# JoelTankard/web-rwkv-gguf

Measured on AMD Instinct MI355X. Metric: tokens/sec RWKV-7 1.5B Q4_K_M decode @1 GPU; achieved HBM GB/s vs roofline, higher is better.
Workload: dtype f16; 1 GPU; RWKV-7 World 1.5B Q4_K_M (Q4_K matrices, Q6_K head, F16 LoRA) batch=1 greedy decode, fused kernels under hipGraph; decode_engine=on, streams_per_gpu=1, pipelines_per_gpu=1, streams=1, parallelism=single

## Files before the change

### web-rwkv-gguf_amd/csrc/wrk_v7_engine.h

```cpp
#pragma once
#include <stdint.h>

#include "wrk_internal.h"

namespace wrk {

constexpr int ENG_K1_JOBS = 7;
constexpr uint32_t ENG_NO_HEAD = 0xffffffffu;

struct EngJob {
    uint32_t rows, row_bytes, f16;
    uint32_t act, mix;
    uint32_t wg0, nwg, rows_per_wg;
    uint32_t gbase;
    uint32_t headed;
};

struct EngShape {
    uint32_t D, F, H, nwg;
    uint32_t rw, ra, rg, rv;
    uint32_t rb_d, rb_f;
    uint32_t rb_w2, rb_a2, rb_g2, rb_v2;
    EngJob k1[ENG_K1_JOBS];
    uint32_t k3_rpw, k5_rpw, k6_rpw;
    uint32_t lds_slot1, lds_slot5, lds_slot6, lds_slot3, lds_xraw0, lds_xraw1, lds_xs, lds_ln, lds_misc, lds_total;
    uint32_t g_x, g_k1, g_o, g_x1, g_k, g_total, g_aux;
    float ln_eps, gn_eps, l2_eps;
    uint32_t layer_begin, layer_end, rescale;
    uint32_t batch, state_rows;
    uint32_t x_from_granules;
};

struct EngLayer {
    const uint8_t *w_r, *w_k, *w_v, *w1, *a1, *g1, *v1;
    const uint8_t *w2, *a2, *g2, *v2;
    const uint8_t *w_o, *ffn_k, *ffn_v;
};
enum { ENG_V_LN1W, ENG_V_LN1B, ENG_V_LN2W, ENG_V_LN2B, ENG_V_MIX0, ENG_V_W0 = ENG_V_MIX0 + 6, ENG_V_A0, ENG_V_V0, ENG_V_RK, ENG_V_KK, ENG_V_KA,
       ENG_V_GNW, ENG_V_GNB, ENG_V_FFNXK, ENG_NV };
enum { ENG_S_O = ENG_K1_JOBS, ENG_S_FK, ENG_S_FV, ENG_NS = 16 };

struct EngArgs {
    EngShape S;
    const EngLayer* layers;
    const void* vecs;
    const float* scal;
    unsigned long long* gran;
    const void* x_in;
    const uint32_t* x_row;
    void* x_out;
    void* v_first;
    float* state;
    uint32_t num_batch;
    uint32_t* fail;
    unsigned long long* stamps;
    uint32_t stamp_layer;
};
constexpr int ENG_STAMPS = 32;

constexpr __host__ __device__ uint32_t eng_wave_pairs(uint32_t pairs, uint32_t ncw, uint32_t wave) {
    const uint32_t simd_rank = (wave + 4u - (ncw + 2u) % 4u) % 4u;
    return pairs / ncw + ((wave / 4u) * 4u + simd_rank < pairs % ncw ? 1u : 0u);
}
constexpr __host__ __device__ uint32_t eng_wave_first_pair(uint32_t pairs, uint32_t ncw, uint32_t wave) {
    const uint32_t extra = pairs % ncw, g4 = (wave / 4u) * 4u;
    uint32_t first = wave * (pairs / ncw) + (extra < g4 ? extra : g4);
    for (uint32_t w = g4; w < wave; ++w) first += eng_wave_pairs(pairs, ncw, w) - pairs / ncw;
    return first;
}
constexpr __host__ __device__ void eng_wave_rows(uint32_t nrows, uint32_t ncw, uint32_t wave, uint32_t& begin, uint32_t& end) {
    const uint32_t pairs = (nrows + 1u) / 2u;
    const uint32_t first = eng_wave_first_pair(pairs, ncw, wave), last = first + eng_wave_pairs(pairs, ncw, wave);
    begin = 2u * first < nrows ? 2u * first : nrows;
    end = 2u * last < nrows ? 2u * last : nrows;
}
constexpr bool eng_wave_rows_ok(uint32_t ncw) {
    for (uint32_t nrows = 0; nrows <= 128; nrows += 2) {
        const uint32_t pairs = nrows / 2, most = (pairs + ncw - 1) / ncw;
// ... 33 lines not shown
```

### web-rwkv-gguf_amd/csrc/wrk_v7_engine.hip

```cpp
#include "wrk_device.h"
#include "wrk_v7.h"
#include "wrk_dmv_body.h"
#include "wrk_v7_engine.h"
#include "wrk_lora_dev.h"

#include <algorithm>
#include <string>

namespace wrk {

#define ENG_LDS __attribute__((address_space(3)))
typedef ENG_LDS unsigned char lds_u8;

#define ENG_BAR() asm volatile("s_waitcnt lgkmcnt(0)\n\ts_barrier" ::: "memory")

constexpr uint32_t ENG_SPIN_MAX = 1u << 21;

__device__ __forceinline__ uint32_t eng_tag(uint32_t layer, uint32_t stage) { return layer * 8u + stage + 1u; }

__device__ __forceinline__ void eng_store_granule(unsigned long long* g, uint32_t tag, uint32_t payload) {
    __hip_atomic_store(g, ((unsigned long long)tag << 32) | payload, __ATOMIC_RELAXED, __HIP_MEMORY_SCOPE_AGENT);
}
__device__ __forceinline__ uint32_t pack_h2(float a, float b) {
    const f16x2 h = {(f16)a, (f16)b};
// ... 105 lines not shown
    const f16x8 z = {0, 0, 0, 0, 0, 0, 0, 0};
    r.v[0] = r.v[1] = r.v[2] = r.v[3] = z;
    r.s[0] = r.s[1] = 0.0f;
    uint32_t lo, hi;
    chunk_xoff<KIND>(c, lo, hi);
    r.v[0] = *(const ENG_LDS f16x8*)(x + lo);
    if (KIND != WRK_MAT_F16) {
        r.v[1] = *(const ENG_LDS f16x8*)(x + lo + 8);
        r.v[2] = *(const ENG_LDS f16x8*)(x + hi);
        r.v[3] = *(const ENG_LDS f16x8*)(x + hi + 8);
    }
    return r;
}

template <int MAXCH>
__device__ __forceinline__ float eng_lora_dot(const f16x8 (&w)[MAXCH], const ENG_LDS f16* aux, uint32_t rank, uint32_t part) {
    float acc = 0.0f;
#pragma unroll
    for (int n = 0; n < MAXCH; ++n) {
        const uint32_t c = part * 8 + 32 * n;
        if (c < rank) {
            const f16x8 x = *(const ENG_LDS f16x8*)(aux + c);
            acc = __builtin_amdgcn_fdot2(__builtin_shufflevector(w[n], w[n], 0, 1), __builtin_shufflevector(x, x, 0, 1), acc, false);
            acc = __builtin_amdgcn_fdot2(__builtin_shufflevector(w[n], w[n], 2, 3), __builtin_shufflevector(x, x, 2, 3), acc, false);
            acc = __builtin_amdgcn_fdot2(__builtin_shufflevector(w[n], w[n], 4, 5), __builtin_shufflevector(x, x, 4, 5), acc, false);
            acc = __builtin_amdgcn_fdot2(__builtin_shufflevector(w[n], w[n], 6, 7), __builtin_shufflevector(x, x, 6, 7), acc, false);
        }
    }
    acc += dpp_f32<0xB1>(acc);
    acc += dpp_f32<0x4E>(acc);
    return acc;
}

struct EngFin {
    uint32_t act;
    float scale;
    const ENG_LDS f16* res;
    float post;
};
__device__ __forceinline__ float eng_finish(const EngFin& f, uint32_t row, float v) {
    float o = act_apply(f.act, v * f.scale);
    if (f.res) o = r16(o) + (float)f.res[row];
    return o;
}

template <int KIND, bool R16, int XI, int RB, class GIDX>
__device__ __forceinline__ void eng_rows(const lds_u8* slot, uint32_t row_bytes, uint32_t K, const ENG_LDS f16* xs, uint32_t row0, uint32_t r_begin,
                                         uint32_t r_end, const EngFin& fin, ENG_LDS uint32_t* pub, unsigned long long* gran, uint32_t tag, GIDX gidx,
                                         uint32_t lane) {
    if (r_begin >= r_end) return;
    const uint32_t kpad = (K + 15u) & ~15u;
    const uint32_t nch = num_chunks<KIND>(K, kpad);
    XRegs x[1][XI];
#pragma unroll
    for (int ci = 0; ci < XI; ++ci) {
        const uint32_t c = lane + 64u * ci;
        x[0][ci] = lds_x<KIND>(xs, min(c, nch - 1));
        if (c >= nch) {
            const f16x8 z = {0, 0, 0, 0, 0, 0, 0, 0};
            x[0][ci].v[0] = x[0][ci].v[1] = x[0][ci].v[2] = x[0][ci].v[3] = z;
        }
        x_sums<KIND>(x[0][ci]);
    }
    static_assert(RB == 2 || RB == 4, "rows per batch");
    constexpr bool PAD = XI > 1;
    for (uint32_t ri = r_begin; ri < r_end; ri += RB) {
// ... 3 lines not shown
        for (int rb = 0; rb < RB; ++rb) {
            const lds_u8* rowp = slot + (size_t)min(ri + rb, r_end - 1) * row_bytes;
#pragma unroll
            for (int ci = 0; ci < XI; ++ci) raw[rb][ci] = lds_raw<KIND>(rowp, K, min(lane + 64u * ci, nch - 1));
        }
        float v[4] = {0.0f, 0.0f, 0.0f, 0.0f};
#pragma unroll
        for (int rb = 0; rb < RB; ++rb)
            if (rb < 2 || whole) {
                float acc[1] = {0.0f};
#pragma unroll
                for (int ci = 0; ci < XI; ++ci) dot_raw_tokens<KIND, R16, 1, XI>(raw[rb][ci], min(lane + 64u * ci, nch - 1), x, ci, acc);
                v[rb] = wave_sum(acc[0]);
            }
        if (lane < RB / 2) {
            const uint32_t ra = ri + 2 * lane;
            if (ra < r_end) {
                const float o0 = eng_finish(fin, row0 + ra, lane ? v[2] : v[0]) * fin.post;
                const float o1 = eng_finish(fin, row0 + ra + 1, lane ? v[3] : v[1]) * fin.post;
                if (pub) pub[ra >> 1] = pack_h2(o0, o1);
                else eng_store_granule(gran + gidx(row0 + ra), tag, pack_h2(o0, o1));
            }
        }
    }
}

template <class GIDX>
__device__ __forceinline__ void eng_publish(const ENG_LDS uint32_t* pub, uint32_t nrows, uint32_t row0, unsigned long long* gran, uint32_t tag, GIDX gidx,
                                            uint32_t lane) {
    for (uint32_t i = lane; 2 * i < nrows; i += 64) eng_store_granule(gran + gidx(row0 + 2 * i), tag, pub[i]);
}

template <int VPT>
__device__ __forceinline__ void eng_ln_mix(bool active, const ENG_LDS f16* xraw, ENG_LDS f16* xs, ENG_LDS f16* ln_out, ENG_LDS float* red, uint32_t K, float eps,
                                           const f16x8 (&wv)[VPT], const f16x8 (&bv)[VPT], const f16x8 (&mv)[VPT], const f32x4 (&pv)[VPT][2],
                                           uint32_t tid, uint32_t lane, uint32_t wave) {
    const uint32_t nvec = K >> 3;
    f16x8 xv[VPT];
    float c0 = 0.0f;
    if (active) {
#pragma unroll
        for (int v = 0; v < VPT; ++v) xv[v] = *(const ENG_LDS f16x8*)(xraw + min(tid + 256u * v, nvec - 1) * 8);
        c0 = (float)xraw[0];
        float s1 = 0.0f, s2 = 0.0f;
#pragma unroll
        for (int v = 0; v < VPT; ++v)
            if (tid + 256u * v < nvec)
#pragma unroll
                for (int e = 0; e < 8; ++e) { const float dl = (float)xv[v][e] - c0; s1 += dl; s2 = __builtin_fmaf(dl, dl, s2); }
        s1 = wave_sum(s1);
        s2 = wave_sum(s2);
        if (lane == 0) { red[wave] = s1; red[4 + wave] = s2; }
    }
    ENG_BAR();
    if (active) {
        const float a1 = (red[0] + red[1]) + (red[2] + red[3]);
        const float a2 = (red[4] + red[5]) + (red[6] + red[7]);
        const float md = a1 / (float)K;
        const float mean = c0 + md;
        const float dev = 1.0f / sqrtf(fmaxf(a2 / (float)K - md * md, 0.0f) + eps);
#pragma unroll
        for (int v = 0; v < VPT; ++v) {
            const uint32_t i = tid + 256u * v;
            if (i >= nvec) continue;
            f16x8 yv, o;
#pragma unroll
            for (int e = 0; e < 8; ++e) {
                yv[e] = (f16)__builtin_fmaf(((float)xv[v][e] - mean) * dev, (float)wv[v][e], (float)bv[v][e]);
                o[e] = (f16)wgsl_mix((float)yv[e], pv[v][e >> 2][e & 3], (float)mv[v][e]);
            }
            *(ENG_LDS f16x8*)(xs + i * 8) = o;
            *(ENG_LDS f16x8*)(ln_out + i * 8) = yv;
        }
    }
    ENG_BAR();
}

constexpr int ENG_LN_BARRIERS = 2;
constexpr int ENG_K1_BARRIERS = 2 + ENG_LN_BARRIERS;
constexpr int ENG_K2_BARRIERS = 6;
constexpr int ENG_K2_CHECKED = 2;
constexpr int ENG_K3_BARRIERS = 2;
constexpr int ENG_K5_BARRIERS = 3 + ENG_LN_BARRIERS;
constexpr int ENG_K6_BARRIERS = 3;
template <int N>
__device__ __forceinline__ void eng_replay() {
#pragma unroll
    for (int i = 0; i < N; ++i) ENG_BAR();
}
template <int XD, bool R16, int QK, int NCW>
__global__ void __launch_bounds__((NCW + 2) * 64) v7_engine_kernel(const EngArgs A, const uint32_t* __restrict__ wg_head) {
    extern __shared__ __attribute__((aligned(16))) unsigned char eng_smem_generic[];
    lds_u8* smem = (lds_u8*)eng_smem_generic;
// ... 134 lines not shown
            ENG_BAR();
            if (*abort_flag) break;
            eng_replay<ENG_K6_BARRIERS - 1>();
            ENG_FLUSH(l);
        }
        return;
    }

    constexpr int VPT = XD;
    constexpr int S64 = 64;
    constexpr int MAXU = (16 + NCW - 1) / NCW;
    const uint32_t nvec = D >> 3;
    const float eps = S.ln_eps;
    const bool ln_wave = wave < 4;
    const uint32_t c0 = is_head ? head * S64 : 0u;
    float vfirst_keep = 0.0f;
    if (is_head && S.layer_begin > 0 && wave == 0) vfirst_keep = (float)((const f16*)A.v_first)[c0 + (tid_all & 63u)];

    unsigned long long clk0 = 0, rt0 = 0;
    if (A.stamps && wg == 0 && tid_all == 0) { clk0 = __builtin_amdgcn_s_memtime(); rt0 = __builtin_amdgcn_s_memrealtime(); }
    for (uint32_t l = S.layer_begin; l < S.layer_end; ++l) {
        uint32_t tid = tid_all;
        asm volatile("" : "+v"(tid));
        const uint32_t lane = tid & 63u;
        float* lst = layer_state(l);
        const bool layer0 = l == 0;
        const f16* lv_base = (const f16*)A.vecs + (size_t)l * ENG_NV * D;
        auto lvec = [&](uint32_t idx) { return lv_base + (size_t)idx * D; };
        const float* scl = A.scal + (size_t)l * ENG_NS;
        const float sc_k1 = scl[j1 < ENG_K1_JOBS ? j1 : 0u], sc_o = scl[ENG_S_O], sc_fk = scl[ENG_S_FK], sc_fv = scl[ENG_S_FV];

        f16x8 wv[VPT], bv[VPT], mv[VPT];
        f32x4 pv[VPT][2];
        if (ln_wave) {
            const f16* mixp = lvec(ENG_V_MIX0 + (j1 < ENG_K1_JOBS ? S.k1[j1].mix : 0u));
#pragma unroll
            for (int v = 0; v < VPT; ++v) {
                const uint32_t i = min(tid + 256u * v, nvec - 1);
                wv[v] = *(const f16x8*)(lvec(ENG_V_LN1W) + i * 8);
                bv[v] = *(const f16x8*)(lvec(ENG_V_LN1B) + i * 8);
                mv[v] = *(const f16x8*)(mixp + i * 8);
                pv[v][0] = *(const f32x4*)(lst + i * 8);
                pv[v][1] = *(const f32x4*)(lst + i * 8 + 4);
            }
        }

        auto request_k5 = [&]() {
            if (ln_wave) {
                float* rowf = lst + (size_t)(srows - 1) * D;
    #pragma unroll
                for (int v = 0; v < VPT; ++v) {
                    const uint32_t i = min(tid + 256u * v, nvec - 1);
                    wv[v] = *(const f16x8*)(lvec(ENG_V_LN2W) + i * 8);
                    bv[v] = *(const f16x8*)(lvec(ENG_V_LN2B) + i * 8);
                    mv[v] = *(const f16x8*)(lvec(ENG_V_FFNXK) + i * 8);
                    pv[v][0] = *(const f32x4*)(rowf + i * 8);
                    pv[v][1] = *(const f32x4*)(rowf + i * 8 + 4);
                }
            }
        };
        if (!is_head) {
            ENG_BAR();
            if (*abort_flag) break;
            ENG_STAMP0(l, 1);
            eng_ln_mix<VPT>(ln_wave, xraw0, xs, lnbuf, red, D, eps, wv, bv, mv, pv, tid, lane, wave);
            ENG_STAMP0(l, 2);
            if (k1_active(l)) {
                const EngJob& J = S.k1[j1];
                uint32_t rb, re;
                eng_wave_rows(k1_rows, NCW, wave, rb, re);
                const EngFin fin{J.act, sc_k1, nullptr, 1.0f};
                const lds_u8* slot = smem + S.lds_slot1;
                ENG_LDS uint32_t* nopub = nullptr;
                if (J.f16) {
                    const uint32_t gb = S.g_k1 + J.gbase;
                    eng_rows<WRK_MAT_F16, false, 4 * XD, 2>(slot, k1_rb, D, xs, k1_row0, rb, re, fin, nopub, A.gran, eng_tag(l, 0),
                                                            [&](uint32_t r) { return gb + (r >> 1); }, lane);
                } else {
                    const uint32_t gb = S.g_k1 + S.g_aux + J.gbase * 32u;
                    eng_rows<QK, R16, XD, 4>(slot, k1_rb, D, xs, k1_row0, rb, re, fin, nopub, A.gran, eng_tag(l, 0),
                                             [&](uint32_t r) { return gb + (r >> 6) * 96u + ((r & 63u) >> 1); }, lane);
                }
            }
            ENG_STAMP0(l, 3);
            ENG_BAR();
        } else {
            const EngLayer& Lp = A.layers[l];
            const uint8_t* p_m[4] = {Lp.w2, Lp.a2, Lp.g2, layer0 ? Lp.w2 : Lp.v2};
            const uint32_t rbm[4] = {S.rb_w2, S.rb_a2, S.rb_g2, layer0 ? S.rb_w2 : S.rb_v2};
            const uint32_t rkm[4] = {S.rw, S.ra, S.rg, layer0 ? S.rw : S.rv};
            f16x8 lu[MAXU][8];
#pragma unroll
            for (int i = 0; i < MAXU; ++i) {
                const uint32_t u = min(wave + (uint32_t)i * NCW, 15u), mi = u >> 2, bi = u & 3u;
                const f16* rowp = (const f16*)(p_m[mi] + (size_t)(c0 + 16u * bi + (lane >> 2)) * rbm[mi]);
#pragma unroll
                for (int n = 0; n < 8; ++n) lu[i][n] = *(const f16x8*)(rowp + min((lane & 3u) * 8 + 32 * n, rkm[mi] - 8));
            }
            float Sreg[16];
            const uint32_t ci64 = tid & 63u, g4 = tid >> 6;
            float* st = lst + (size_t)D + c0 + ci64;
            if (ln_wave) {
#pragma unroll
                for (int jj = 0; jj < 16; ++jj) Sreg[jj] = st[(size_t)(g4 * 16 + jj) * D];
            }
            f16 h_w0 = 0, h_a0 = 0, h_kk = 0, h_ka = 0, h_v0 = 0, h_gnw = 0, h_gnb = 0, h_rk = 0;
            if (wave == 0) {
                const uint32_t cc = c0 + lane;
                h_w0 = lvec(ENG_V_W0)[cc]; h_a0 = lvec(ENG_V_A0)[cc]; h_kk = lvec(ENG_V_KK)[cc]; h_ka = lvec(ENG_V_KA)[cc]; h_v0 = lvec(ENG_V_V0)[cc];
                h_gnw = lvec(ENG_V_GNW)[cc]; h_gnb = lvec(ENG_V_GNB)[cc]; h_rk = lvec(ENG_V_RK)[cc];
            }
            ENG_BAR();
            if (*abort_flag) break;
            ENG_STAMP0(l, 1);
            eng_ln_mix<VPT>(ln_wave, xraw0, xs, lnbuf, red, D, eps, wv, bv, mv, pv, tid, lane, wave);
            ENG_STAMP0(l, 3);
            ENG_BAR();

            ENG_LDS float* sh_r = k2f; ENG_LDS float* sh_w = k2f + 64; ENG_LDS float* sh_k = k2f + 128; ENG_LDS float* sh_v = k2f + 192;
            ENG_LDS float* sh_a = k2f + 256; ENG_LDS float* sh_b = k2f + 320; ENG_LDS float* sh_g = k2f + 384; ENG_LDS float* sh_kk = k2f + 448;
            ENG_LDS float* sh_red = k2f + 512;
            ENG_LDS float* sh_red2 = k2f + 768;
            ENG_LDS float* sh_d = k2f + 1024;
            ENG_BAR();
            if (*abort_flag) break;
            ENG_STAMP0(l, 4);
            {
                const ENG_LDS f16* auxm[4] = {auxbuf, auxbuf + S.rw, auxbuf + S.rw + S.ra, layer0 ? auxbuf : auxbuf + S.rw + S.ra + S.rg};
#pragma unroll
                for (int i = 0; i < MAXU; ++i) {
                    const uint32_t u = wave + (uint32_t)i * NCW;
                    if (u < 16u) {
                        const uint32_t mi = u >> 2, bi = u & 3u;
                        const float dd = eng_lora_dot<8>(lu[i], auxm[mi], rkm[mi], lane & 3u);
                        if ((lane & 3u) == 0) sh_d[mi * 64 + 16 * bi + (lane >> 2)] = dd;
                    }
                }
            }
            ENG_STAMP0(l, 16);
            ENG_BAR();
            if (abort_flag[1]) break;
            const ENG_LDS f16* hr = auxbuf + naux, *hk = hr + 64, *hv = hr + 128;
            if (wave == 0) {
                const float w0 = (float)h_w0, a0 = (float)h_a0, kkw = (float)h_kk, kaw = (float)h_ka;
                const float kraw = (float)hk[lane], rraw = (float)hr[lane];
                float v = (float)hv[lane];
                const float v0w = layer0 ? 0.0f : (float)h_v0, vfirst = layer0 ? 0.0f : vfirst_keep;
                const float dw = sh_d[lane], da = sh_d[64 + lane], dg = sh_d[128 + lane], dv = layer0 ? 0.0f : sh_d[192 + lane];
                const float w = r16(w0 + r16(dw));
                const float a = r16(act_sigmoid(a0 + r16(da)));
                const float g = r16(dg);
                if (layer0) { vfirst_keep = v; ((f16*)A.v_first)[c0 + lane] = (f16)v; }
                else {
                    const float vv = r16(act_sigmoid(v0w + r16(dv)));
                    v = r16(wgsl_mix(v, vfirst, vv));
                }
                sh_w[lane] = __expf(-0.606531f * act_sigmoid(w));
                sh_g[lane] = g;
                sh_v[lane] = v;
                sh_r[lane] = rraw;
                const float kkv = r16(kkw * kraw);
                sh_k[lane] = r16(kraw * (1.0f + (a - 1.0f) * kaw));
                const float nrm = 1.0f / sqrtf(wave_sum(kkv * kkv) + S.l2_eps);
                const float kkn = r16(kkv * nrm);
                sh_a[lane] = -kkn;
                sh_b[lane] = kkn * a;
                sh_kk[lane] = kkv;
// ... 148 lines not shown
            const float o_next = __shfl_down(o, 1, WAVE);
            if (valid) {
                lst[(size_t)(srows - 1) * D + r] = (float)lnbuf[r];
                if ((lane & 1u) == 0) eng_store_granule(A.gran + S.g_x + (r >> 1), eng_tag(l, 4), pack_h2(o, o_next));
                if (l + 1 == S.layer_end) ((f16*)A.x_out)[r] = (f16)o;
            }
        }
        ENG_STAMP0(l, 13);
        ENG_BAR();
        ENG_FLUSH(l);
    }
    if (A.stamps && wg == 0 && tid_all == 0) {
        unsigned long long* tail = A.stamps + (size_t)S.nwg * 16 * 24;
        tail[0] = __builtin_amdgcn_s_memtime() - clk0;
        tail[1] = __builtin_amdgcn_s_memrealtime() - rt0;
    }
#undef ENG_STAMP
#undef ENG_STAMP0
#undef ENG_FLUSH
}

}

struct wrk_v7_engine {
    wrk_v7_model* m = nullptr;
    wrk::EngShape S{};
    wrk::EngLayer* layers = nullptr;
    void* vecs = nullptr;
    float* scal = nullptr;
    uint32_t* wg_head = nullptr;
    unsigned long long* gran = nullptr;
    uint32_t* fail = nullptr;
    unsigned long long* stamps = nullptr;
    void* emb_ln = nullptr;
    bool r16 = false;
    int xd = 1, ncw = 8;
    uint32_t quant = 0;
};

static uint32_t up(uint32_t v, uint32_t a) { return (v + a - 1) / a * a; }

typedef void (*eng_fn)(const wrk::EngArgs, const uint32_t*);
static eng_fn eng_kernel(int xd, bool r16, int ncw) {
    using namespace wrk;
#define ENG_PICK(XD_, R_) (ncw == 14 ? (eng_fn)v7_engine_kernel<XD_, R_, WRK_MAT_Q4_K, 14> : (eng_fn)v7_engine_kernel<XD_, R_, WRK_MAT_Q4_K, 8>)
    if (xd == 1) return r16 ? ENG_PICK(1, true) : ENG_PICK(1, false);
    return r16 ? ENG_PICK(2, true) : ENG_PICK(2, false);
#undef ENG_PICK
}
static const void* eng_kernel_fn(int xd, bool r16, int ncw) { return (const void*)eng_kernel(xd, r16, ncw); }

int32_t wrk_v7_engine_create(wrk_v7_model* m, wrk_v7_engine** out) {
    using namespace wrk;
    wrk_ctx* ctx = m->ctx;
    *out = nullptr;
    const auto& d = m->d;
    const uint32_t D = d.num_emb, F = d.num_hidden, H = d.num_head, NWG = (uint32_t)ctx->num_cu;
    auto no = [&](const char* why) { return wrk_fail(ctx, WRK_E_UNSUPPORTED, "decode engine: %s", why); };
    if (m->act_dtype != WRK_F16) return no("f32 frames");
    if (H == 0 || D != H * 64 || D % 256 || D > 4096 || F % 1024 || F != 4 * D) return no("shape");
    if (d.lora_w % 8 || d.lora_a % 8 || d.lora_g % 8 || d.lora_v % 8 || d.lora_w < 8 || d.lora_a < 8 || d.lora_g < 8 || d.lora_v < 8 ||
        d.lora_w > 128 || d.lora_a > 128 || d.lora_v > 128 || d.lora_g > 256 || ((d.lora_w + d.lora_a + d.lora_g + d.lora_v) % 16))
        return no("LoRA ranks");
    if (NWG < 2 * H || NWG < 64) return no("too few compute units");
    uint32_t quant = 0xffffffffu, flags = 0xffffffffu;
    for (size_t li = 0; li < m->layers.size(); ++li) {
        const auto& L = m->layers[li];
        const wrk_matrix* big[] = {L.w_r, L.w_k, L.w_v, L.w_o, L.ffn_w_k, L.ffn_w_v};
        for (const wrk_matrix* q : big) {
            if (quant == 0xffffffffu) { quant = q->kind; flags = q->flags; }
            if (q->kind != quant || q->flags != flags) return no("mixed matrix kinds");
        }
        const wrk_matrix* lo[] = {L.w1, L.a1, L.g1, li ? L.v1 : L.a1, L.w2, L.a2, L.g2, li ? L.v2 : L.a2};
        for (const wrk_matrix* q : lo)
            if (!q || q->kind != WRK_MAT_F16) return no("LoRA matrices must be F16");
        if (L.w_r->k != D || L.w_r->m != D || L.ffn_w_k->m != F || L.ffn_w_v->k != F || L.w1->m != d.lora_w || L.a1->m != d.lora_a ||
            L.g1->m != d.lora_g || (li && L.v1->m != d.lora_v))
            return no("matrix shapes");
    }
    if (quant != WRK_MAT_Q4_K) return no("only Q4_K matrices so far");
    if (m->layers.empty()) return no("no layers");

    wrk_v7_engine* e = new wrk_v7_engine();
    e->m = m;
    e->quant = quant;
    e->r16 = (flags & WRK_MATRIX_ROUND_F16) != 0;
    e->xd = D <= 2048 ? 1 : 2;
    EngShape& S = e->S;
    S.D = D; S.F = F; S.H = H; S.nwg = NWG;
    S.rw = d.lora_w; S.ra = d.lora_a; S.rg = d.lora_g; S.rv = d.lora_v;
    const auto& L0 = m->layers[0];
    const auto& L1 = m->layers[m->layers.size() > 1 ? 1 : 0];
    S.rb_d = (uint32_t)L0.w_r->row_bytes; S.rb_f = (uint32_t)L0.ffn_w_v->row_bytes;
    S.rb_w2 = (uint32_t)L0.w2->row_bytes; S.rb_a2 = (uint32_t)L0.a2->row_bytes; S.rb_g2 = (uint32_t)L0.g2->row_bytes;
    S.rb_v2 = (uint32_t)(m->layers.size() > 1 ? L1.v2->row_bytes : L0.a2->row_bytes);
    for (const auto& L : m->layers) {
        if (L.w_r->row_bytes != S.rb_d || L.w_k->row_bytes != S.rb_d || L.w_v->row_bytes != S.rb_d || L.w_o->row_bytes != S.rb_d ||
            L.ffn_w_k->row_bytes != S.rb_d || L.ffn_w_v->row_bytes != S.rb_f || L.w2->row_bytes != S.rb_w2 || L.a2->row_bytes != S.rb_a2 ||
            L.g2->row_bytes != S.rb_g2) { delete e; return no("row strides differ between layers"); }
    }
    const uint32_t rb_l = (uint32_t)L0.w1->row_bytes;
    struct { uint32_t rows, rb, f16, act, mix, headed, gbase; } jd[ENG_K1_JOBS] = {
        {D, S.rb_d, 0, WRK_ACT_NONE, 0, 1, 0}, {D, S.rb_d, 0, WRK_ACT_NONE, 2, 1, 1}, {D, S.rb_d, 0, WRK_ACT_NONE, 3, 1, 2},
        {S.rw, rb_l, 1, WRK_ACT_TANH, 1, 0, 0}, {S.ra, rb_l, 1, WRK_ACT_NONE, 4, 0, S.rw / 2}, {S.rg, rb_l, 1, WRK_ACT_SIGMOID, 5, 0, (S.rw + S.ra) / 2},
        {S.rv, rb_l, 1, WRK_ACT_NONE, 3, 0, (S.rw + S.ra + S.rg) / 2}};
    double total = 0;
    for (auto& j : jd) total += (double)j.rows * j.rb;
    uint32_t slot1 = 0;
    bool placed = false;
    const uint32_t NK1 = NWG - H;
    for (double target = total / NK1; target < total; target *= 1.03) {
        uint32_t used = 0, worst = 0;
        uint32_t rpw[ENG_K1_JOBS], nw[ENG_K1_JOBS];
        for (int j = 0; j < ENG_K1_JOBS; ++j) {
            uint32_t r = (uint32_t)(target / jd[j].rb);
            r = std::max(2u, r / 2 * 2);
            rpw[j] = r;
            nw[j] = (jd[j].rows + r - 1) / r;
            used += nw[j];
            worst = std::max(worst, std::min(r, jd[j].rows) * jd[j].rb);
        }
        if (used > NK1) continue;
        uint32_t w0 = 0;
        for (int j = 0; j < ENG_K1_JOBS; ++j) {
            S.k1[j] = EngJob{jd[j].rows, jd[j].rb, jd[j].f16, jd[j].act, jd[j].mix, w0, nw[j], rpw[j], jd[j].gbase, jd[j].headed};
            w0 += nw[j];
        }
        slot1 = worst;
        placed = true;
        break;
    }
    if (!placed) { delete e; return no("K1 partition"); }
// ... 11 lines not shown
    S.lds_xraw1 = take(D * 2);
    const uint32_t naux = S.rw + S.ra + S.rg + S.rv;
    S.lds_ln = take(D * 2);
    S.lds_misc = take(4096);
    S.lds_xs = take(D * 2 + up((naux + 192) * 2, 16) + 1280 * 4);
    int lds_max = 0;
    hipDeviceGetAttribute(&lds_max, hipDeviceAttributeMaxSharedMemoryPerBlock, ctx->device);
    if (lds_max < 160 * 1024) lds_max = 160 * 1024;
    if (off > (uint32_t)lds_max) { delete e; return no("weights of a layer do not fit the LDS"); }
    S.lds_total = std::max(off, S.lds_xs + F * 2);
    if (S.lds_total > (uint32_t)lds_max) { delete e; return no("the ffn vector's exchange area does not fit the LDS behind a layer's weights"); }
    S.g_aux = naux / 2;
    uint32_t g = 0;
    auto gtake = [&](uint32_t n) { const uint32_t o = g; g += up(n, 128); return o; };
    S.g_x = gtake(D / 2);
    S.g_k1 = gtake(S.g_aux + H * 96);
    S.g_o = gtake(D / 2);
    S.g_x1 = gtake(D / 2);
    S.g_k = gtake(F / 2);
    S.g_total = g;
    S.ln_eps = 1.0e-5f; S.gn_eps = 64.0e-5f; S.l2_eps = 1.0e-12f;
    S.rescale = d.rescale ? d.rescale : 0xffffffffu;
    S.state_rows = 64 + 2;

    std::vector<float> hs(m->layers.size() * ENG_NS, 1.0f);
    auto fail_alloc = [&](hipError_t er) { wrk_v7_engine_destroy(e); return wrk_fail(ctx, WRK_E_OOM, "decode engine: %s", hipGetErrorString(er)); };
    hipError_t er;
    std::vector<EngLayer> hl(m->layers.size());
    for (size_t li = 0; li < m->layers.size(); ++li) {
        const auto& L = m->layers[li];
        EngLayer& o = hl[li];
        o.w_r = L.w_r->data; o.w_k = L.w_k->data; o.w_v = L.w_v->data; o.w1 = L.w1->data; o.a1 = L.a1->data; o.g1 = L.g1->data;
        o.v1 = li ? L.v1->data : L.a1->data;
        o.w2 = L.w2->data; o.a2 = L.a2->data; o.g2 = L.g2->data; o.v2 = li ? L.v2->data : L.a2->data;
        o.w_o = L.w_o->data; o.ffn_k = L.ffn_w_k->data; o.ffn_v = L.ffn_w_v->data;
        const wrk_matrix* k1m[ENG_K1_JOBS] = {L.w_r, L.w_k, L.w_v, L.w1, L.a1, L.g1, li ? L.v1 : L.a1};
        float* sc = hs.data() + li * ENG_NS;
        for (int j = 0; j < ENG_K1_JOBS; ++j) sc[j] = k1m[j]->out_scale;
        sc[ENG_S_O] = L.w_o->out_scale; sc[ENG_S_FK] = L.ffn_w_k->out_scale; sc[ENG_S_FV] = L.ffn_w_v->out_scale;
    }
    if ((er = hipMalloc((void**)&e->vecs, hl.size() * ENG_NV * D * 2)) != hipSuccess) return fail_alloc(er);
    for (size_t li = 0; li < m->layers.size(); ++li) {
        const auto& L = m->layers[li];
        const wrk_buf* src[ENG_NV] = {L.ln1_w, L.ln1_b, L.ln2_w, L.ln2_b, L.x_r, L.x_w, L.x_k, L.x_v, L.x_a, L.x_g, L.w0, L.a0, li ? L.v0 : L.w0,
                                      L.r_k, L.k_k, L.k_a, L.gn_w, L.gn_b, L.ffn_x_k};
        for (int i = 0; i < ENG_NV; ++i) {
            if (!src[i] || src[i]->bytes < (size_t)D * 2) { wrk_v7_engine_destroy(e); return no("a layer vector is missing"); }
            if ((er = hipMemcpy((char*)e->vecs + (li * ENG_NV + i) * (size_t)D * 2, src[i]->ptr, (size_t)D * 2, hipMemcpyDeviceToDevice)) != hipSuccess) return fail_alloc(er);
        }
    }
    if ((er = hipMalloc((void**)&e->scal, hs.size() * 4)) != hipSuccess) return fail_alloc(er);
    if ((er = hipMemcpy(e->scal, hs.data(), hs.size() * 4, hipMemcpyHostToDevice)) != hipSuccess) return fail_alloc(er);
    if ((er = hipMalloc((void**)&e->layers, hl.size() * sizeof(EngLayer))) != hipSuccess) return fail_alloc(er);
    if ((er = hipMemcpy(e->layers, hl.data(), hl.size() * sizeof(EngLayer), hipMemcpyHostToDevice)) != hipSuccess) return fail_alloc(er);
    std::vector<uint32_t> hh(2 * NWG, ENG_NO_HEAD);
    for (uint32_t h = 0; h < H; ++h) hh[2 * ((size_t)h * NWG / H)] = h;
    for (uint32_t w = 0, r = 0; w < NWG; ++w)
        if (hh[2 * w] == ENG_NO_HEAD) hh[2 * w + 1] = r++;
    if ((er = hipMalloc((void**)&e->wg_head, hh.size() * 4)) != hipSuccess) return fail_alloc(er);
    if ((er = hipMemcpy(e->wg_head, hh.data(), hh.size() * 4, hipMemcpyHostToDevice)) != hipSuccess) return fail_alloc(er);
    if ((er = hipMalloc((void**)&e->gran, (size_t)S.g_total * 8)) != hipSuccess) return fail_alloc(er);
    if ((er = hipMalloc((void**)&e->fail, 256)) != hipSuccess) return fail_alloc(er);
    if ((er = hipMemset(e->fail, 0, 256)) != hipSuccess) return fail_alloc(er);
    const char* tm = getenv("WRK_TIMING");
    if (tm && tm[0] == '1') {
        const size_t n = (size_t)NWG * 16 * 24 * 8 + 64;
        if ((er = hipMalloc((void**)&e->stamps, n)) != hipSuccess) return fail_alloc(er);
        hipMemset(e->stamps, 0, n);
    }
    { const char* ev = getenv("WRK_ENGINE_WAVES"); e->ncw = (ev && atoi(ev) == 14) ? 14 : 8; }
    const void* fn = eng_kernel_fn(e->xd, e->r16, e->ncw);
    if ((er = hipFuncSetAttribute(fn, hipFuncAttributeMaxDynamicSharedMemorySize, (int)S.lds_total)) != hipSuccess) {
        wrk_v7_engine_destroy(e);
        return wrk_fail(ctx, WRK_E_UNSUPPORTED, "decode engine: %u bytes of LDS refused (%s)", S.lds_total, hipGetErrorString(er));
    }
    {
        hipFuncAttributes fa{};
        const int waves = e->ncw + 2, per_simd = (waves + 3) / 4;
        if (hipFuncGetAttributes(&fa, fn) == hipSuccess && fa.numRegs > 0) {
            const int alloc = (fa.numRegs + 7) / 8 * 8;
            if (per_simd * alloc > 512 || fa.maxThreadsPerBlock < waves * 64 || (size_t)fa.sharedSizeBytes + S.lds_total > 160 * 1024) {
                const int regs = fa.numRegs;
                wrk_v7_engine_destroy(e);
                return wrk_fail(ctx, WRK_E_UNSUPPORTED, "decode engine: a workgroup of %d waves x %d registers + %u bytes of LDS does not fit a CU", waves, regs,
                                S.lds_total);
            }
        }
        (void)hipGetLastError();
    }
    {
        const char* te = getenv("WRK_ENGINE_TABLE");
        if (!(te && te[0] == '0') && m->emb && m->ln0_w && m->ln0_b) {
            const size_t bytes = (size_t)d.num_vocab * D * 2;
            if (hipMalloc(&e->emb_ln, bytes) == hipSuccess) {
                LnMixParams P{};
                P.src = (const f16*)m->emb->ptr; P.ln_w = (const f16*)m->ln0_w->ptr; P.ln_b = (const f16*)m->ln0_b->ptr; P.eps = 1.0e-5f;
                P.d = D; P.nmix = 0; P.ln_out = (f16*)e->emb_ln;
                if (ln_mix(ctx->stream, P, d.num_vocab) != 0 || hipStreamSynchronize(ctx->stream) != hipSuccess) { hipFree(e->emb_ln); e->emb_ln = nullptr; }
            } else e->emb_ln = nullptr;
            (void)hipGetLastError();
        }
    }
    *out = e;
    return WRK_OK;
}

bool wrk_v7_engine_has_table(const wrk_v7_engine* e) { return e && e->emb_ln; }
int wrk_v7_engine_waves(const wrk_v7_engine* e) { return e ? e->ncw : 0; }

void wrk_v7_engine_destroy(wrk_v7_engine* e) {
    if (!e) return;
    if (e->emb_ln) hipFree(e->emb_ln);
    if (e->layers) hipFree(e->layers);
    if (e->vecs) hipFree(e->vecs);
    if (e->scal) hipFree(e->scal);
    if (e->wg_head) hipFree(e->wg_head);
    if (e->gran) hipFree(e->gran);
    if (e->fail) hipFree(e->fail);
    if (e->stamps) hipFree(e->stamps);
    delete e;
}

int32_t wrk_v7_engine_enqueue(wrk_v7_engine* e, hipStream_t q, wrk_v7_state* st, uint32_t batch, uint32_t l0, uint32_t l1, const void* x_in, void* x_out,
                              void* v_first, const uint32_t* token) {
    using namespace wrk;
    wrk_ctx* ctx = e->m->ctx;
    EngArgs A{};
    A.S = e->S;
    A.S.layer_begin = l0; A.S.layer_end = l1; A.S.batch = batch;
    A.layers = e->layers; A.vecs = e->vecs; A.scal = e->scal; A.gran = e->gran; A.x_in = x_in; A.x_out = x_out; A.v_first = v_first;
    if (token && e->emb_ln && l0 == 0) { A.x_in = e->emb_ln; A.x_row = token; }
    A.state = st->data; A.num_batch = st->num_batch; A.fail = e->fail; A.stamps = e->stamps; A.stamp_layer = std::min(5u, l1 - 1);
    WRK_HIP(ctx, hipMemsetAsync(e->gran, 0, (size_t)e->S.g_total * 8, q));
    const dim3 grid(e->S.nwg), block((e->ncw + 2) * 64);
    hipLaunchKernelGGL(eng_kernel(e->xd, e->r16, e->ncw), grid, block, e->S.lds_total, q, A, (const uint32_t*)e->wg_head);
    WRK_LAUNCH_CHECK(ctx);
    return WRK_OK;
}

int32_t wrk_v7_engine_check(wrk_v7_engine* e) {
    if (!e) return WRK_OK;
    wrk_ctx* ctx = e->m->ctx;
    uint32_t f = 0;
    WRK_HIP(ctx, hipMemcpy(&f, e->fail, 4, hipMemcpyDeviceToHost));
    if (f) {
        hipMemset(e->fail, 0, 4);
        return wrk_fail(ctx, WRK_E_HIP, "decode engine: a hand-off wait gave up (stage mask 0x%x): workgroups not co-resident or a producer died", f);
    }
    return WRK_OK;
}

void wrk_v7_engine_report(wrk_v7_engine* e) {
    using namespace wrk;
    if (!e || !e->stamps) return;
    const uint32_t NWG = e->S.nwg, NW = (uint32_t)e->ncw + 2;
    std::vector<unsigned long long> h((size_t)NWG * NW * 24);
    if (hipMemcpy(h.data(), e->stamps, h.size() * 8, hipMemcpyDeviceToHost) != hipSuccess) return;
    unsigned long long t0 = ~0ull;
    for (auto v : h) if (v && v < t0) t0 = v;
    std::vector<char> is_head(NWG, 0);
    for (uint32_t hd = 0; hd < e->S.H; ++hd) is_head[(size_t)hd * NWG / e->S.H] = 1;
    auto col = [&](int wave, uint32_t k, const char* label, int cls = -1) {
        std::vector<double> v;
        for (uint32_t w = 0; w < NWG; ++w) {
            if (cls >= 0 && is_head[w] != cls) continue;
            unsigned long long x = 0;
            if (wave >= 0) x = h[((size_t)w * NW + wave) * 24 + k];
            else for (int cw = 0; cw < e->ncw; ++cw) x = std::max(x, h[((size_t)w * NW + cw) * 24 + k]);
            if (x) v.push_back((double)(x - t0) * 0.01);
        }
        if (v.empty()) return;
        std::sort(v.begin(), v.end());
        fprintf(stderr, "  %-62s %4zu WGs  first %7.2f  median %7.2f  last %7.2f us\n", label, v.size(), v.front(), v[v.size() / 2], v.back());
    };
    {
        unsigned long long tail[2] = {0, 0};
        if (hipMemcpy(tail, e->stamps + (size_t)NWG * 16 * 24, 16, hipMemcpyDeviceToHost) == hipSuccess && tail[1])
            fprintf(stderr, "[WRK_TIMING] decode engine: shader clock over the last launch %.0f MHz (%llu cycles in %.1f us)\n",
                    (double)tail[0] / ((double)tail[1] * 0.01), tail[0], (double)tail[1] * 0.01);
    }
    const int G = e->ncw, Ld = e->ncw + 1;
    fprintf(stderr, "[WRK_TIMING] decode engine (%d compute waves), one layer of the last token; us since the layer's first stamp\n", e->ncw);
    col(G, 0, "gather: layer input complete, workgroups without a head", 0);
    col(G, 0, "gather: layer input complete, head workgroups", 1);
    col(0, 1, "K1 start (input + weights in LDS), wave 0, no head", 0);
    col(0, 1, "K1 start (input in LDS), wave 0, head workgroups", 1);
    col(0, 2, "K1 LN + shift done, wave 0");
    col(0, 3, "K1 rows published, wave 0, no head", 0);
    col(-1, 3, "K1 rows published, slowest wave, no head", 0);
    col(-1, 3, "K1 LN + shift done, slowest wave, head workgroups", 1);
    col(G, 4, "gather (heads): LoRA intermediates complete");
    col(G, 1, "gather (heads): K1 outputs complete");
    col(0, 4, "K2 start");
    col(-1, 16, "K2 LoRA dots done, slowest wave");
    col(0, 17, "K2 per-channel stage done");
    col(-1, 18, "K2 state updated, slowest wave");
    col(0, 5, "K2 published");
    col(G, 2, "gather: head outputs complete");
    col(0, 6, "K3 start");
    col(-1, 7, "K3 published, slowest wave");
    col(G, 3, "gather: x1 complete");
    col(0, 8, "K5 start");
    col(0, 14, "K5 LN + shift done, wave 0");
    col(0, 9, "K5 published, wave 0");
    col(-1, 9, "K5 published, slowest wave");
    col(0, 10, "K6 own quarter of the ffn vector swept, wave 0");
    col(-1, 10, "K6 swept, slowest wave");
    col(0, 11, "K6 start");
    col(-1, 15, "K6 inputs read back from LDS, slowest wave");
    col(-1, 12, "K6 partial sums done, slowest wave");
    col(0, 13, "K6 published");
    col(Ld, 0, "loader: K1 slot free, next layer's fill issued");
}
```

Before: 1781 tokens/s.

## Pre-pack LoRA up-projection weights per head for coalesced lane-contiguous loads

At engine creation the LoRA up-projection matrices (w2, a2, g2, v2) are repacked into 1 KB pieces per head and unit, so each lane reads 16 contiguous bytes and only as many pieces as the rank needs. This replaces strided row loads, which were clamped to the rank and re-read overlapping data. The head workgroups also skip the full LN+mix preload and compute only their own 64 LN outputs with a per-lane LN weight and bias. The cost is an extra device buffer, plus a host round-trip to repack every layer at startup.

```diff
diff --git a/web-rwkv-gguf_amd/csrc/wrk_lora2_pack.h b/web-rwkv-gguf_amd/csrc/wrk_lora2_pack.h
--- /dev/null
+++ b/web-rwkv-gguf_amd/csrc/wrk_lora2_pack.h
@@ -0,0 +1,80 @@
+#pragma once
+#include <stddef.h>
+#include <stdint.h>
+
+#ifndef WRK_HD
+#ifdef __HIPCC__
+#define WRK_HD __host__ __device__
+#else
+#define WRK_HD
+#endif
+#endif
+
+namespace wrk {
+
+constexpr uint32_t ENG_L2_PIECE_BYTES = 1024;
+constexpr uint32_t ENG_L2_UNITS = 16;
+constexpr uint32_t ENG_L2_MAX_PIECES = 8;
+
+struct EngLora2Ranks { uint32_t w, a, g, v; };
+WRK_HD constexpr uint32_t eng_l2_rank(const EngLora2Ranks& R, uint32_t m) { return m == 0u ? R.w : m == 1u ? R.a : m == 2u ? R.g : R.v; }
+WRK_HD constexpr uint32_t eng_l2_pieces(uint32_t rank) { return (rank + 31u) / 32u; }
+WRK_HD constexpr uint32_t eng_l2_unit_piece(const EngLora2Ranks& R, uint32_t u) {
+    const uint32_t m = u / 4u;
+    const uint32_t whole = (m > 0u ? eng_l2_pieces(R.w) : 0u) + (m > 1u ? eng_l2_pieces(R.a) : 0u) + (m > 2u ? eng_l2_pieces(R.g) : 0u) +
+                           (m > 3u ? eng_l2_pieces(R.v) : 0u);
+    return 4u * whole + (u % 4u) * eng_l2_pieces(eng_l2_rank(R, m));
+}
+WRK_HD constexpr uint32_t eng_l2_head_pieces(const EngLora2Ranks& R) { return eng_l2_unit_piece(R, ENG_L2_UNITS); }
+WRK_HD constexpr size_t eng_l2_piece(const EngLora2Ranks& R, uint32_t head, uint32_t u, uint32_t n) {
+    return (size_t)head * eng_l2_head_pieces(R) + eng_l2_unit_piece(R, u) + n;
+}
+WRK_HD constexpr size_t eng_l2_layer_bytes(const EngLora2Ranks& R, uint32_t heads) {
+    return (size_t)heads * eng_l2_head_pieces(R) * ENG_L2_PIECE_BYTES;
+}
+WRK_HD constexpr uint32_t eng_l2_src_row(uint32_t head, uint32_t u, uint32_t lane) { return head * 64u + 16u * (u % 4u) + lane / 4u; }
+WRK_HD constexpr uint32_t eng_l2_src_col(uint32_t n, uint32_t lane) { return 8u * (lane % 4u) + 32u * n; }
+
+constexpr bool eng_l2_layout_ok() {
+    for (uint32_t rank = 8; rank <= 256; rank += 8) {
+        const uint32_t np = eng_l2_pieces(rank);
+        if (np == 0 || np > ENG_L2_MAX_PIECES || 32u * (np - 1u) >= rank || 32u * np < rank) return false;
+        for (uint32_t c = 0; c < rank; c += 8) {
+            uint32_t owners = 0;
+            for (uint32_t n = 0; n < np; ++n)
+                for (uint32_t q = 0; q < 4; ++q) owners += eng_l2_src_col(n, q) == c ? 1u : 0u;
+            if (owners != 1) return false;
+        }
+        for (uint32_t pos = 0; pos < 4; ++pos) {
+            const EngLora2Ranks R{pos == 0 ? rank : 96u, pos == 1 ? rank : 40u, pos == 2 ? rank : 256u, pos == 3 ? rank : 8u};
+            uint32_t next = 0;
+            for (uint32_t u = 0; u < ENG_L2_UNITS; ++u) {
+                if (eng_l2_unit_piece(R, u) != next) return false;
+                next += eng_l2_pieces(eng_l2_rank(R, u / 4u));
+            }
+            if (eng_l2_head_pieces(R) != next || eng_l2_piece(R, 3, 0, 0) != 3u * next) return false;
+        }
+    }
+    for (uint32_t lane = 0; lane < 64; ++lane)
+        if (eng_l2_src_row(2, 7, lane) != 2u * 64u + 48u + lane / 4u) return false;
+    return true;
+}
+static_assert(eng_l2_layout_ok(), "LoRA-2 pack: a column without exactly one (piece, lane), or units that are not dense and in order");
+static_assert(eng_l2_head_pieces(EngLora2Ranks{96, 96, 256, 64}) == 64, "LoRA-2 pack: pieces of a 1.5B head");
+
+inline void eng_l2_pack_layer(const EngLora2Ranks& R, uint32_t heads, const uint8_t* const (&src)[4], const size_t (&row_bytes)[4], uint8_t* dst) {
+    for (uint32_t head = 0; head < heads; ++head)
+        for (uint32_t u = 0; u < ENG_L2_UNITS; ++u) {
+            const uint32_t m = u / 4u, rank = eng_l2_rank(R, m);
+            for (uint32_t n = 0; n < eng_l2_pieces(rank); ++n) {
+                uint8_t* piece = dst + eng_l2_piece(R, head, u, n) * ENG_L2_PIECE_BYTES;
+                for (uint32_t lane = 0; lane < 64; ++lane) {
+                    const uint32_t c = eng_l2_src_col(n, lane);
+                    for (uint32_t b = 0; b < 16; ++b)
+                        piece[16u * lane + b] = (src[m] && c < rank) ? src[m][(size_t)eng_l2_src_row(head, u, lane) * row_bytes[m] + 2u * c + b] : 0;
+                }
+            }
+        }
+}
+
+}
diff --git a/web-rwkv-gguf_amd/csrc/wrk_v7_engine.h b/web-rwkv-gguf_amd/csrc/wrk_v7_engine.h
--- a/web-rwkv-gguf_amd/csrc/wrk_v7_engine.h
+++ b/web-rwkv-gguf_amd/csrc/wrk_v7_engine.h
@@ -2,6 +2,7 @@
 #include <stdint.h>
 
 #include "wrk_internal.h"
+#include "wrk_lora2_pack.h"
 
 namespace wrk {
 
@@ -20,7 +21,6 @@
     uint32_t D, F, H, nwg;
     uint32_t rw, ra, rg, rv;
     uint32_t rb_d, rb_f;
-    uint32_t rb_w2, rb_a2, rb_g2, rb_v2;
     EngJob k1[ENG_K1_JOBS];
     uint32_t k3_rpw, k5_rpw, k6_rpw;
     uint32_t lds_slot1, lds_slot5, lds_slot6, lds_slot3, lds_xraw0, lds_xraw1, lds_xs, lds_ln, lds_misc, lds_total;
@@ -33,7 +33,6 @@
 
 struct EngLayer {
     const uint8_t *w_r, *w_k, *w_v, *w1, *a1, *g1, *v1;
-    const uint8_t *w2, *a2, *g2, *v2;
     const uint8_t *w_o, *ffn_k, *ffn_v;
 };
 enum { ENG_V_LN1W, ENG_V_LN1B, ENG_V_LN2W, ENG_V_LN2B, ENG_V_MIX0, ENG_V_W0 = ENG_V_MIX0 + 6, ENG_V_A0, ENG_V_V0, ENG_V_RK, ENG_V_KK, ENG_V_KA,
@@ -44,6 +43,7 @@
     EngShape S;
     const EngLayer* layers;
     const void* vecs;
+    const uint8_t* l2;
     const float* scal;
     unsigned long long* gran;
     const void* x_in;
diff --git a/web-rwkv-gguf_amd/csrc/wrk_v7_engine.hip b/web-rwkv-gguf_amd/csrc/wrk_v7_engine.hip
--- a/web-rwkv-gguf_amd/csrc/wrk_v7_engine.hip
+++ b/web-rwkv-gguf_amd/csrc/wrk_v7_engine.hip
@@ -161,6 +161,15 @@
     return acc;
 }
 
+template <int NP>
+__device__ __forceinline__ void eng_l2_load(f16x8 (&w)[8], const uint8_t* up) {
+#pragma unroll
+    for (int n = 0; n < NP; ++n) w[n] = *(const f16x8*)(up + n * ENG_L2_PIECE_BYTES);
+    const f16x8 z = {0, 0, 0, 0, 0, 0, 0, 0};
+#pragma unroll
+    for (int n = NP; n < 8; ++n) w[n] = z;
+}
+
 struct EngFin {
     uint32_t act;
     float scale;
@@ -230,33 +239,45 @@
 }
 
 template <int VPT>
+__device__ __forceinline__ void eng_ln_partial(bool active, const ENG_LDS f16* xraw, ENG_LDS float* red, uint32_t K, f16x8 (&xv)[VPT], float& c0, uint32_t tid,
+                                               uint32_t lane, uint32_t wave) {
+    const uint32_t nvec = K >> 3;
+    c0 = 0.0f;
+    if (active) {
+#pragma unroll
+        for (int v = 0; v < VPT; ++v) xv[v] = *(const ENG_LDS f16x8*)(xraw + min(tid + 256u * v, nvec - 1) * 8);
+        c0 = (float)xraw[0];
+        float s1 = 0.0f, s2 = 0.0f;
+#pragma unroll
+        for (int v = 0; v < VPT; ++v)
+            if (tid + 256u * v < nvec)
+#pragma unroll
+                for (int e = 0; e < 8; ++e) { const float dl = (float)xv[v][e] - c0; s1 += dl; s2 = __builtin_fmaf(dl, dl, s2); }
+        s1 = wave_sum(s1);
+        s2 = wave_sum(s2);
+        if (lane == 0) { red[wave] = s1; red[4 + wave] = s2; }
+    }
+}
+__device__ __forceinline__ void eng_ln_stats(const ENG_LDS float* red, float c0, uint32_t K, float eps, float& mean, float& dev) {
+    const float a1 = (red[0] + red[1]) + (red[2] + red[3]);
+    const float a2 = (red[4] + red[5]) + (red[6] + red[7]);
+    const float md = a1 / (float)K;
+    mean = c0 + md;
+    dev = 1.0f / sqrtf(fmaxf(a2 / (float)K - md * md, 0.0f) + eps);
+}
+
+template <int VPT>
 __device__ __forceinline__ void eng_ln_mix(bool active, const ENG_LDS f16* xraw, ENG_LDS f16* xs, ENG_LDS f16* ln_out, ENG_LDS float* red, uint32_t K, float eps,
                                            const f16x8 (&wv)[VPT], const f16x8 (&bv)[VPT], const f16x8 (&mv)[VPT], const f32x4 (&pv)[VPT][2],
                                            uint32_t tid, uint32_t lane, uint32_t wave) {
     const uint32_t nvec = K >> 3;
     f16x8 xv[VPT];
-    float c0 = 0.0f;
-    if (active) {
-#pragma unroll
-        for (int v = 0; v < VPT; ++v) xv[v] = *(const ENG_LDS f16x8*)(xraw + min(tid + 256u * v, nvec - 1) * 8);
-        c0 = (float)xraw[0];
-        float s1 = 0.0f, s2 = 0.0f;
-#pragma unroll
-        for (int v = 0; v < VPT; ++v)
-            if (tid + 256u * v < nvec)
-#pragma unroll
-                for (int e = 0; e < 8; ++e) { const float dl = (float)xv[v][e] - c0; s1 += dl; s2 = __builtin_fmaf(dl, dl, s2); }
-        s1 = wave_sum(s1);
-        s2 = wave_sum(s2);
-        if (lane == 0) { red[wave] = s1; red[4 + wave] = s2; }
-    }
+    float c0;
+    eng_ln_partial<VPT>(active, xraw, red, K, xv, c0, tid, lane, wave);
     ENG_BAR();
     if (active) {
-        const float a1 = (red[0] + red[1]) + (red[2] + red[3]);
-        const float a2 = (red[4] + red[5]) + (red[6] + red[7]);
-        const float md = a1 / (float)K;
-        const float mean = c0 + md;
-        const float dev = 1.0f / sqrtf(fmaxf(a2 / (float)K - md * md, 0.0f) + eps);
+        float mean, dev;
+        eng_ln_stats(red, c0, K, eps, mean, dev);
 #pragma unroll
         for (int v = 0; v < VPT; ++v) {
             const uint32_t i = tid + 256u * v;
@@ -457,7 +478,7 @@
 
         f16x8 wv[VPT], bv[VPT], mv[VPT];
         f32x4 pv[VPT][2];
-        if (ln_wave) {
+        if (ln_wave && !is_head) {
             const f16* mixp = lvec(ENG_V_MIX0 + (j1 < ENG_K1_JOBS ? S.k1[j1].mix : 0u));
 #pragma unroll
             for (int v = 0; v < VPT; ++v) {
@@ -510,17 +531,27 @@
             ENG_STAMP0(l, 3);
             ENG_BAR();
         } else {
-            const EngLayer& Lp = A.layers[l];
-            const uint8_t* p_m[4] = {Lp.w2, Lp.a2, Lp.g2, layer0 ? Lp.w2 : Lp.v2};
-            const uint32_t rbm[4] = {S.rb_w2, S.rb_a2, S.rb_g2, layer0 ? S.rb_w2 : S.rb_v2};
-            const uint32_t rkm[4] = {S.rw, S.ra, S.rg, layer0 ? S.rw : S.rv};
+            f16 h_lnw = 0, h_lnb = 0;
+            if (wave == 1) { h_lnw = lvec(ENG_V_LN1W)[c0 + lane]; h_lnb = lvec(ENG_V_LN1B)[c0 + lane]; }
+            const EngLora2Ranks R2{S.rw, S.ra, S.rg, S.rv};
+            const uint8_t* l2_head = A.l2 + (l * eng_l2_layer_bytes(R2, S.H) + eng_l2_piece(R2, head, 0, 0) * ENG_L2_PIECE_BYTES);
             f16x8 lu[MAXU][8];
 #pragma unroll
             for (int i = 0; i < MAXU; ++i) {
-                const uint32_t u = min(wave + (uint32_t)i * NCW, 15u), mi = u >> 2, bi = u & 3u;
-                const f16* rowp = (const f16*)(p_m[mi] + (size_t)(c0 + 16u * bi + (lane >> 2)) * rbm[mi]);
-#pragma unroll
-                for (int n = 0; n < 8; ++n) lu[i][n] = *(const f16x8*)(rowp + min((lane & 3u) * 8 + 32 * n, rkm[mi] - 8));
+                const uint32_t u = wave + (uint32_t)i * NCW;
+                const uint32_t np = u < ENG_L2_UNITS ? eng_l2_pieces(eng_l2_rank(R2, u >> 2)) : 0u;
+                const uint8_t* up = l2_head + (eng_l2_unit_piece(R2, u) * ENG_L2_PIECE_BYTES + lane * 16u);
+                switch (np) {
+                    case 1: eng_l2_load<1>(lu[i], up); break;
+                    case 2: eng_l2_load<2>(lu[i], up); break;
+                    case 3: eng_l2_load<3>(lu[i], up); break;
+                    case 4: eng_l2_load<4>(lu[i], up); break;
+                    case 5: eng_l2_load<5>(lu[i], up); break;
+                    case 6: eng_l2_load<6>(lu[i], up); break;
+                    case 7: eng_l2_load<7>(lu[i], up); break;
+                    case 8: eng_l2_load<8>(lu[i], up); break;
+                    default: eng_l2_load<0>(lu[i], up); break;
+                }
             }
             float Sreg[16];
             const uint32_t ci64 = tid & 63u, g4 = tid >> 6;
@@ -535,10 +566,24 @@
                 h_w0 = lvec(ENG_V_W0)[cc]; h_a0 = lvec(ENG_V_A0)[cc]; h_kk = lvec(ENG_V_KK)[cc]; h_ka = lvec(ENG_V_KA)[cc]; h_v0 = lvec(ENG_V_V0)[cc];
                 h_gnw = lvec(ENG_V_GNW)[cc]; h_gnb = lvec(ENG_V_GNB)[cc]; h_rk = lvec(ENG_V_RK)[cc];
             }
+            ENG_STAMP0(l, 19);
             ENG_BAR();
             if (*abort_flag) break;
             ENG_STAMP0(l, 1);
-            eng_ln_mix<VPT>(ln_wave, xraw0, xs, lnbuf, red, D, eps, wv, bv, mv, pv, tid, lane, wave);
+            {
+                f16x8 xv[VPT];
+                float x0;
+                eng_ln_partial<VPT>(ln_wave, xraw0, red, D, xv, x0, tid, lane, wave);
+                ENG_BAR();
+                if (wave == 1) {
+                    float mean, dev;
+                    eng_ln_stats(red, x0, D, eps, mean, dev);
+                    float y = __builtin_fmaf(((float)xraw0[c0 + lane] - mean) * dev, (float)h_lnw, (float)h_lnb);
+                    asm volatile("" : "+v"(y));
+                    lnbuf[c0 + lane] = (f16)y;
+                }
+                ENG_BAR();
+            }
             ENG_STAMP0(l, 3);
             ENG_BAR();
 
@@ -557,7 +602,7 @@
                     const uint32_t u = wave + (uint32_t)i * NCW;
                     if (u < 16u) {
                         const uint32_t mi = u >> 2, bi = u & 3u;
-                        const float dd = eng_lora_dot<8>(lu[i], auxm[mi], rkm[mi], lane & 3u);
+                        const float dd = eng_lora_dot<8>(lu[i], auxm[mi], eng_l2_rank(R2, mi), lane & 3u);
                         if ((lane & 3u) == 0) sh_d[mi * 64 + 16 * bi + (lane >> 2)] = dd;
                     }
                 }
@@ -772,6 +817,7 @@
     unsigned long long* gran = nullptr;
     uint32_t* fail = nullptr;
     unsigned long long* stamps = nullptr;
+    uint8_t* l2pack = nullptr;
     void* emb_ln = nullptr;
     bool r16 = false;
     int xd = 1, ncw = 8;
@@ -815,7 +861,8 @@
         for (const wrk_matrix* q : lo)
             if (!q || q->kind != WRK_MAT_F16) return no("LoRA matrices must be F16");
         if (L.w_r->k != D || L.w_r->m != D || L.ffn_w_k->m != F || L.ffn_w_v->k != F || L.w1->m != d.lora_w || L.a1->m != d.lora_a ||
-            L.g1->m != d.lora_g || (li && L.v1->m != d.lora_v))
+            L.g1->m != d.lora_g || (li && L.v1->m != d.lora_v) || L.w2->k != d.lora_w || L.a2->k != d.lora_a || L.g2->k != d.lora_g ||
+            (li && L.v2->k != d.lora_v) || L.w2->m != D || L.a2->m != D || L.g2->m != D || (li && L.v2->m != D))
             return no("matrix shapes");
     }
     if (quant != WRK_MAT_Q4_K) return no("only Q4_K matrices so far");
@@ -830,14 +877,10 @@
     S.D = D; S.F = F; S.H = H; S.nwg = NWG;
     S.rw = d.lora_w; S.ra = d.lora_a; S.rg = d.lora_g; S.rv = d.lora_v;
     const auto& L0 = m->layers[0];
-    const auto& L1 = m->layers[m->layers.size() > 1 ? 1 : 0];
     S.rb_d = (uint32_t)L0.w_r->row_bytes; S.rb_f = (uint32_t)L0.ffn_w_v->row_bytes;
-    S.rb_w2 = (uint32_t)L0.w2->row_bytes; S.rb_a2 = (uint32_t)L0.a2->row_bytes; S.rb_g2 = (uint32_t)L0.g2->row_bytes;
-    S.rb_v2 = (uint32_t)(m->layers.size() > 1 ? L1.v2->row_bytes : L0.a2->row_bytes);
     for (const auto& L : m->layers) {
         if (L.w_r->row_bytes != S.rb_d || L.w_k->row_bytes != S.rb_d || L.w_v->row_bytes != S.rb_d || L.w_o->row_bytes != S.rb_d ||
-            L.ffn_w_k->row_bytes != S.rb_d || L.ffn_w_v->row_bytes != S.rb_f || L.w2->row_bytes != S.rb_w2 || L.a2->row_bytes != S.rb_a2 ||
-            L.g2->row_bytes != S.rb_g2) { delete e; return no("row strides differ between layers"); }
+            L.ffn_w_k->row_bytes != S.rb_d || L.ffn_w_v->row_bytes != S.rb_f) { delete e; return no("row strides differ between layers"); }
     }
     const uint32_t rb_l = (uint32_t)L0.w1->row_bytes;
     struct { uint32_t rows, rb, f16, act, mix, headed, gbase; } jd[ENG_K1_JOBS] = {
@@ -915,7 +958,6 @@
         EngLayer& o = hl[li];
         o.w_r = L.w_r->data; o.w_k = L.w_k->data; o.w_v = L.w_v->data; o.w1 = L.w1->data; o.a1 = L.a1->data; o.g1 = L.g1->data;
         o.v1 = li ? L.v1->data : L.a1->data;
-        o.w2 = L.w2->data; o.a2 = L.a2->data; o.g2 = L.g2->data; o.v2 = li ? L.v2->data : L.a2->data;
         o.w_o = L.w_o->data; o.ffn_k = L.ffn_w_k->data; o.ffn_v = L.ffn_w_v->data;
         const wrk_matrix* k1m[ENG_K1_JOBS] = {L.w_r, L.w_k, L.w_v, L.w1, L.a1, L.g1, li ? L.v1 : L.a1};
         float* sc = hs.data() + li * ENG_NS;
@@ -930,6 +972,32 @@
         for (int i = 0; i < ENG_NV; ++i) {
             if (!src[i] || src[i]->bytes < (size_t)D * 2) { wrk_v7_engine_destroy(e); return no("a layer vector is missing"); }
             if ((er = hipMemcpy((char*)e->vecs + (li * ENG_NV + i) * (size_t)D * 2, src[i]->ptr, (size_t)D * 2, hipMemcpyDeviceToDevice)) != hipSuccess) return fail_alloc(er);
+        }
+    }
+    {
+        const EngLora2Ranks R2{S.rw, S.ra, S.rg, S.rv};
+        const size_t lb = eng_l2_layer_bytes(R2, H), total_l2 = lb * m->layers.size();
+        if ((er = hipMalloc((void**)&e->l2pack, total_l2)) != hipSuccess) {
+            (void)hipGetLastError();
+            wrk_v7_engine_destroy(e);
+            return wrk_fail(ctx, WRK_E_UNSUPPORTED, "decode engine: %zu bytes for the packed LoRA up-projections refused (%s)", total_l2, hipGetErrorString(er));
+        }
+        std::vector<uint8_t> img(lb), rows[4];
+        for (size_t li = 0; li < m->layers.size(); ++li) {
+            const auto& L = m->layers[li];
+            const wrk_matrix* mats[4] = {L.w2, L.a2, L.g2, li ? L.v2 : nullptr};
+            const uint8_t* src[4] = {nullptr, nullptr, nullptr, nullptr};
+            size_t rbs[4] = {0, 0, 0, 0};
+            for (int i = 0; i < 4; ++i) {
+                if (!mats[i]) continue;
+                rbs[i] = mats[i]->row_bytes;
+                if (rbs[i] < (size_t)eng_l2_rank(R2, i) * 2) { wrk_v7_engine_destroy(e); return no("a LoRA up-projection's rows are shorter than its rank"); }
+                rows[i].resize((size_t)D * rbs[i]);
+                if ((er = hipMemcpy(rows[i].data(), mats[i]->data, rows[i].size(), hipMemcpyDeviceToHost)) != hipSuccess) return fail_alloc(er);
+                src[i] = rows[i].data();
+            }
+            eng_l2_pack_layer(R2, H, src, rbs, img.data());
+            if ((er = hipMemcpy(e->l2pack + li * lb, img.data(), lb, hipMemcpyHostToDevice)) != hipSuccess) return fail_alloc(er);
         }
     }
     if ((er = hipMalloc((void**)&e->scal, hs.size() * 4)) != hipSuccess) return fail_alloc(er);
@@ -994,6 +1062,7 @@
 void wrk_v7_engine_destroy(wrk_v7_engine* e) {
     if (!e) return;
     if (e->emb_ln) hipFree(e->emb_ln);
+    if (e->l2pack) hipFree(e->l2pack);
     if (e->layers) hipFree(e->layers);
     if (e->vecs) hipFree(e->vecs);
     if (e->scal) hipFree(e->scal);
@@ -1011,7 +1080,7 @@
     EngArgs A{};
     A.S = e->S;
     A.S.layer_begin = l0; A.S.layer_end = l1; A.S.batch = batch;
-    A.layers = e->layers; A.vecs = e->vecs; A.scal = e->scal; A.gran = e->gran; A.x_in = x_in; A.x_out = x_out; A.v_first = v_first;
+    A.layers = e->layers; A.vecs = e->vecs; A.l2 = e->l2pack; A.scal = e->scal; A.gran = e->gran; A.x_in = x_in; A.x_out = x_out; A.v_first = v_first;
     if (token && e->emb_ln && l0 == 0) { A.x_in = e->emb_ln; A.x_row = token; }
     A.state = st->data; A.num_batch = st->num_batch; A.fail = e->fail; A.stamps = e->stamps; A.stamp_layer = std::min(5u, l1 - 1);
     WRK_HIP(ctx, hipMemsetAsync(e->gran, 0, (size_t)e->S.g_total * 8, q));
@@ -1066,6 +1135,7 @@
     fprintf(stderr, "[WRK_TIMING] decode engine (%d compute waves), one layer of the last token; us since the layer's first stamp\n", e->ncw);
     col(G, 0, "gather: layer input complete, workgroups without a head", 0);
     col(G, 0, "gather: layer input complete, head workgroups", 1);
+    col(-1, 19, "operand requests issued, slowest wave, head workgroups", 1);
     col(0, 1, "K1 start (input + weights in LDS), wave 0, no head", 0);
     col(0, 1, "K1 start (input in LDS), wave 0, head workgroups", 1);
     col(0, 2, "K1 LN + shift done, wave 0");
```

Result: faster. 1868 tokens/s, median of 6 (+4.9%).
